# Hippogriff/parsenet-codebase

Measured on AMD Instinct MI355X. Metric: shapes/sec fwd+bwd on 10k-pt clouds, higher is better.
Workload: dtype f32; 1 GPU; cfg5: ParSeNet e2e (seg + mean-shift 10 it. + per-segment spline/primitive fit + Chamfer/residual), 10k pts, batch 4 per GPU, fwd+bwd+allreduce+Adam; batch_per_gpu=4, points=10000, k=80, parallelism=dp1, global_batch=4

## Files before the change

### include/parsenet_hip.h

```cpp
#ifndef PARSENET_HIP_H
#define PARSENET_HIP_H

#include <stddef.h>
#include <stdint.h>

#ifdef __cplusplus
extern "C" {
#endif

#define PN_ABI_VERSION 23

#define PN_OK 0
#define PN_ERR_ARG (-1)
#define PN_ERR_HIP (-2)
#define PN_ERR_WORKSPACE (-3)
#define PN_ERR_UNSUPPORTED (-4)

const char* pn_last_error(void);
int pn_abi_version(void);

void pn_prof_enable(int on);
void pn_prof_reset(void);
int pn_prof_count(void);
int pn_prof_get(int i, char* name, int name_len, double* total_ms, long long* calls);
// ... 74 lines not shown
int pn_gemm_x3_f32(const void* img_a, const float* x, const float* bias, int B, int M, int K, int N, float* out,
                   void* workspace, size_t workspace_bytes, void* stream);
int pn_gemm_x3_cat_f32(const void* img_a, const float* const* xs, const int* cs, int nsrc, const float* bias, int B,
                       int M, int N, float* out, void* workspace, size_t workspace_bytes, void* stream);
size_t pn_gemm_x3_wgrad_workspace(int B, int M, int K, int N);
int pn_gemm_x3_wgrad_f32(const float* gy, const float* x, int B, int M, int K, int N, float* gw, float* gb,
                         void* workspace, size_t workspace_bytes, void* stream);
size_t pn_meanshift_rows_bwd_workspace(int B, int N);
int pn_meanshift_rows_bwd_f32(const float* gy, const float* y, const float* q, const float* rsum, const float* unorm,
                              const float* x, const float* bsq, int B, int N, int D, int R, float* gq, float* gx,
                              void* workspace, size_t workspace_bytes, void* stream);
int pn_meanshift_rows_bwd_kind_f32(const float* gy, const float* y, const float* q, const float* rsum,
                                   const float* unorm, const float* x, const float* bsq, int B, int N, int D, int R,
                                   float* gq, float* gx, void* workspace, size_t workspace_bytes, int kind,
                                   void* stream);
int pn_meanshift_rows_scatter_add_f32(const float* g, const int64_t* rows, int B, int N, int D, int R, float* gx,
                                      void* stream);
size_t pn_meanshift_x3_plan_bytes(int B, int N);
size_t pn_meanshift_x3_plan_core_bytes(int B, int N);
int pn_kmeans_assign_f32(const float* x, const float* cen, int B, int N, int D, int K, int* lab, void* stream);
int pn_kmeans_centres_f32(const float* x, const int* lab, const float* old, int B, int N, int D, int K,
                          float* cen, void* stream);
int pn_cell_order_i32(const int* rank, const int* home, const int* fine, int B, int N, int P, int F,
                      long long* perm, void* stream);
int pn_meanshift_x3_tileinfo_f32(const float* z, int B, int N, int D, float* cen, float* rho, float* cnt,
                                 void* stream);
int pn_meanshift_x3_plan_f32(const float* cenQ, const float* rhoQ, const float* cenX, const float* rhoX,
                             const float* cntX, const float* bsq, int B, int N, float rel_eps, void* plan,
                             void* stream);
int pn_meanshift_x3_iter_fwd_plan_f32(const float* q, const void* img_x, const float* bsq, int B, int N,
// ... 226 lines not shown
```

### parsenet_codebase_amd/csrc/meanshift_rows.hip

```cpp
#include "common.h"
#include <cstdlib>

#define MR_DMAX 128
#define MR_R 64
#define MR_CB 64
#define MR_LDOF(D) ((D) + 4)
#define MR_LG 68
#define MR_LOG2E 1.4426950408889634f
#define MR_LIM2 (75.0f * MR_LOG2E)

__device__ static inline float4 mr_ld4(const float* p) { return *reinterpret_cast<const float4*>(p); }
template <int NV>
__device__ static inline void mr_ldn(const float* p, float* v) {
  if constexpr (NV == 8) {
    const float4 a = mr_ld4(p), b = mr_ld4(p + 4);
    v[0] = a.x; v[1] = a.y; v[2] = a.z; v[3] = a.w;
    v[4] = b.x; v[5] = b.y; v[6] = b.z; v[7] = b.w;
  } else if constexpr (NV == 4) {
    const float4 a = mr_ld4(p);
    v[0] = a.x; v[1] = a.y; v[2] = a.z; v[3] = a.w;
  } else {
    const float2 a = *reinterpret_cast<const float2*>(p);
    v[0] = a.x; v[1] = a.y;
  }
}

template <int MR_D, int MR_LD>
__global__ __launch_bounds__(256) void pn_ms_rows_prep_kernel(const float* __restrict__ gy, const float* __restrict__ y,
                                                              const float* __restrict__ rsum, const float* __restrict__ unorm,
                                                              const float* __restrict__ bsq, int R, float* __restrict__ gu,
                                                              float* __restrict__ scal) {
  const int b = blockIdx.y;
  const int wave = threadIdx.x >> 6, lane = threadIdx.x & 63;
  const int r = blockIdx.x * 4 + wave;
  if (r >= MR_R) return;
  float u0 = 0.f, u1 = 0.f, c = 0.f, al = 0.f, ri = 0.f;
  if (r < R) {
    const size_t base = ((size_t)b * R + r) * MR_D;
    const bool lo = MR_D >= 64 || lane < MR_D;
    float y0 = 0.f, y1 = 0.f, g0 = 0.f, g1 = 0.f;
    if (lo) y0 = y[base + lane];
    if constexpr (MR_D == 128) y1 = y[base + lane + 64];
    if (lo) g0 = gy[base + lane];
    if constexpr (MR_D == 128) g1 = gy[base + lane + 64];
    const float nn = unorm[(size_t)b * R + r], rr = rsum[(size_t)b * R + r];
    const float yg = pn_wave_sum(y0 * g0 + y1 * g1);
    u0 = (g0 - y0 * yg) / nn;
    u1 = (g1 - y1 * yg) / nn;
    c = pn_wave_sum(u0 * (y0 * nn) + u1 * (y1 * nn));
    al = 1.0f / (rr * bsq[b]);
    ri = 1.0f / rr;
  }
  float* g = gu + ((size_t)b * MR_R + r) * MR_D;
  if (lane < MR_D) g[lane] = u0;
  if constexpr (MR_D == 128) g[lane + 64] = u1;
  if (lane == 0) {
    float* sp = scal + ((size_t)b * MR_R + r) * 4;
    sp[0] = c;
    sp[1] = al;
    sp[2] = ri;
    sp[3] = 0.f;
  }
}

template <int MR_D, int MR_LD, int MR_KIND>
__global__ __launch_bounds__(256) void pn_ms_rows_bwd_kernel(
    const float* __restrict__ gu, const float* __restrict__ scal, const float* __restrict__ q,
    const float* __restrict__ x, const float* __restrict__ bsq, int N, int R, int nblk, float* __restrict__ gx,
    float* __restrict__ gq_part) {
  extern __shared__ __attribute__((aligned(16))) float lds[];
  float* Xs = lds;
  float* Qs = Xs + MR_CB * MR_LD;
  float* Us = Qs + MR_R * MR_LD;
  float* GS = Us + MR_R * MR_LD;
  float* KR = GS + MR_R * MR_LG;
  float* GT = KR + MR_R * MR_LG;
  float* sc = GT + MR_CB * MR_LG;
  float* sa = sc + MR_R;
  float* sr = sa + MR_R;
  const int b = blockIdx.y, blk = blockIdx.x, tid = threadIdx.x;
  constexpr int MR_L4 = MR_D == 128 ? 5 : MR_D == 64 ? 4 : 3;

  const int j0 = blk * MR_CB;
  const float bs = bsq[b];
  const float hl = (0.5f / bs) * MR_LOG2E;
  const float ib = 1.0f / bs;
  const float* __restrict__ xb = x + (size_t)b * N * MR_D;

  for (int it = tid; it < MR_CB * (MR_D / 4); it += 256) {
    const int r = it >> MR_L4, c4 = it & (MR_D / 4 - 1);
    float4 v = make_float4(0.f, 0.f, 0.f, 0.f);
    if (j0 + r < N) v = mr_ld4(xb + (size_t)(j0 + r) * MR_D + 4 * c4);
    *reinterpret_cast<float4*>(Xs + r * MR_LD + 4 * c4) = v;
    float4 w = make_float4(0.f, 0.f, 0.f, 0.f);
    if (r < R) w = mr_ld4(q + ((size_t)b * R + r) * MR_D + 4 * c4);
    *reinterpret_cast<float4*>(Qs + r * MR_LD + 4 * c4) = w;
  }
  for (int it = tid; it < MR_R * (MR_D / 4); it += 256) {
    const int r = it >> MR_L4, c4 = it & (MR_D / 4 - 1);
    *reinterpret_cast<float4*>(Us + r * MR_LD + 4 * c4) = mr_ld4(gu + ((size_t)b * MR_R + r) * MR_D + 4 * c4);
  }
  if (tid < MR_R) {
    const float4 sv = mr_ld4(scal + ((size_t)b * MR_R + tid) * 4);
    sc[tid] = sv.x;
    sa[tid] = sv.y;
    sr[tid] = sv.z;
  }
  __syncthreads();

  {
    const int ti = tid >> 4, tj = tid & 15;
    float s[4][4], t[4][4];
#pragma unroll
    for (int a = 0; a < 4; ++a)
#pragma unroll
      for (int e = 0; e < 4; ++e) {
        s[a][e] = 0.f;
        t[a][e] = 0.f;
      }
    for (int k = 0; k < MR_D; k += 4) {
      float4 qv[4], uv[4], xv[4];
#pragma unroll
      for (int a = 0; a < 4; ++a) {
        qv[a] = mr_ld4(Qs + (ti + 16 * a) * MR_LD + k);
        uv[a] = mr_ld4(Us + (ti + 16 * a) * MR_LD + k);
        xv[a] = mr_ld4(Xs + (tj + 16 * a) * MR_LD + k);
      }
#pragma unroll
      for (int a = 0; a < 4; ++a)
#pragma unroll
        for (int e = 0; e < 4; ++e) {
          s[a][e] = __builtin_fmaf(qv[a].x, xv[e].x, s[a][e]);
          s[a][e] = __builtin_fmaf(qv[a].y, xv[e].y, s[a][e]);
          s[a][e] = __builtin_fmaf(qv[a].z, xv[e].z, s[a][e]);
          s[a][e] = __builtin_fmaf(qv[a].w, xv[e].w, s[a][e]);
          t[a][e] = __builtin_fmaf(uv[a].x, xv[e].x, t[a][e]);
          t[a][e] = __builtin_fmaf(uv[a].y, xv[e].y, t[a][e]);
          t[a][e] = __builtin_fmaf(uv[a].z, xv[e].z, t[a][e]);
          t[a][e] = __builtin_fmaf(uv[a].w, xv[e].w, t[a][e]);
        }
    }
#pragma unroll
    for (int a = 0; a < 4; ++a) {
      const int i = ti + 16 * a;
      const float ci = sc[i], ai = sa[i], ri = sr[i];
#pragma unroll
      for (int e = 0; e < 4; ++e) {
        const int j = tj + 16 * e;
        const float dist = __builtin_fmaf(-2.0f, s[a][e], 2.0f);
        float kv, g;
        if constexpr (MR_KIND == PN_MS_KERNEL_EPANECHNIKOV) {
          kv = fmaxf(0.0f, 0.75f * __builtin_fmaf(-dist, ib, 1.0f));
          if (j0 + j >= N) kv = 0.f;
          g = kv > 0.0f ? 1.5f * ((t[a][e] - ci) * ai) : 0.f;
        } else {
          const float a2 = -dist * hl;
          const float a2c = __builtin_amdgcn_fmed3f(a2, -MR_LIM2, MR_LIM2);
          kv = __builtin_amdgcn_exp2f(a2c);
          if (j0 + j >= N) kv = 0.f;
          g = a2c == a2 ? kv * ((t[a][e] - ci) * ai) : 0.f;
        }
        GS[i * MR_LG + j] = g;
        GT[j * MR_LG + i] = g;
        KR[i * MR_LG + j] = kv * ri;
      }
    }
  }
  __syncthreads();

  constexpr int NF4 = MR_D / 4;
  constexpr int RPT = MR_CB * NF4 / 256;
  const int f4 = tid & (NF4 - 1), grp = tid >> MR_L4;
  {
    float4 acc[RPT];
#pragma unroll
    for (int e = 0; e < RPT; ++e) acc[e] = make_float4(0.f, 0.f, 0.f, 0.f);
    for (int i = 0; i < MR_R; ++i) {
      const float4 qv = mr_ld4(Qs + i * MR_LD + 4 * f4);
      const float4 uv = mr_ld4(Us + i * MR_LD + 4 * f4);
      float gv[RPT], kv[RPT];
      mr_ldn<RPT>(GS + i * MR_LG + RPT * grp, gv);
      mr_ldn<RPT>(KR + i * MR_LG + RPT * grp, kv);
#pragma unroll
      for (int e = 0; e < RPT; ++e) {
        acc[e].x = __builtin_fmaf(gv[e], qv.x, acc[e].x);
        acc[e].y = __builtin_fmaf(gv[e], qv.y, acc[e].y);
        acc[e].z = __builtin_fmaf(gv[e], qv.z, acc[e].z);
        acc[e].w = __builtin_fmaf(gv[e], qv.w, acc[e].w);
        acc[e].x = __builtin_fmaf(kv[e], uv.x, acc[e].x);
        acc[e].y = __builtin_fmaf(kv[e], uv.y, acc[e].y);
        acc[e].z = __builtin_fmaf(kv[e], uv.z, acc[e].z);
        acc[e].w = __builtin_fmaf(kv[e], uv.w, acc[e].w);
      }
    }
#pragma unroll
    for (int e = 0; e < RPT; ++e) {
      const int j = j0 + RPT * grp + e;
      if (j < N) {
        float4* o = reinterpret_cast<float4*>(gx + ((size_t)b * N + j) * MR_D + 4 * f4);
        float4 v = *o;
        v.x += acc[e].x;
        v.y += acc[e].y;
        v.z += acc[e].z;
        v.w += acc[e].w;
        *o = v;
      }
    }
  }
  {
    float4 acc[RPT];
#pragma unroll
    for (int e = 0; e < RPT; ++e) acc[e] = make_float4(0.f, 0.f, 0.f, 0.f);
    for (int j = 0; j < MR_CB; ++j) {
      const float4 xv = mr_ld4(Xs + j * MR_LD + 4 * f4);
      float gv[RPT];
      mr_ldn<RPT>(GT + j * MR_LG + RPT * grp, gv);
#pragma unroll
      for (int e = 0; e < RPT; ++e) {
        acc[e].x = __builtin_fmaf(gv[e], xv.x, acc[e].x);
        acc[e].y = __builtin_fmaf(gv[e], xv.y, acc[e].y);
        acc[e].z = __builtin_fmaf(gv[e], xv.z, acc[e].z);
        acc[e].w = __builtin_fmaf(gv[e], xv.w, acc[e].w);
      }
    }
    float* pb = gq_part + ((size_t)b * nblk + blk) * MR_R * MR_D;
#pragma unroll
    for (int e = 0; e < RPT; ++e) *reinterpret_cast<float4*>(pb + (RPT * grp + e) * MR_D + 4 * f4) = acc[e];
  }
}

template <int MR_D, int MR_LD>
__global__ __launch_bounds__(256) void pn_ms_rows_reduce_kernel(const float* __restrict__ gq_part, int R, int nblk,
                                                                float* __restrict__ gq) {
  const int b = blockIdx.y;
  const int e = blockIdx.x * 256 + threadIdx.x;
  if (e >= R * (MR_D / 4)) return;
  const float* p = gq_part + (size_t)b * nblk * MR_R * MR_D + 4 * e;
  float4 s = make_float4(0.f, 0.f, 0.f, 0.f);
  int k = 0;
  for (; k + 8 <= nblk; k += 8) {
    float4 v[8];
#pragma unroll
    for (int u = 0; u < 8; ++u) v[u] = mr_ld4(p + (size_t)(k + u) * MR_R * MR_D);
#pragma unroll
    for (int u = 0; u < 8; ++u) {
      s.x += v[u].x;
      s.y += v[u].y;
      s.z += v[u].z;
      s.w += v[u].w;
    }
  }
  for (; k < nblk; ++k) {
    const float4 v = mr_ld4(p + (size_t)k * MR_R * MR_D);
    s.x += v.x;
    s.y += v.y;
    s.z += v.z;
    s.w += v.w;
  }
  *reinterpret_cast<float4*>(gq + (size_t)b * R * MR_D + 4 * e) = s;
}

template <int MR_D, int MR_LD>
__global__ __launch_bounds__(256) void pn_ms_rows_scatter_kernel(const float* __restrict__ g, const int64_t* __restrict__ rows,
                                                                 int N, int R, float* __restrict__ gx) {
  const int b = blockIdx.x, tid = threadIdx.x;
  const int f4 = tid & 31, sub = tid >> 5;
  for (int r0 = 0; r0 < R; r0 += 8) {
    for (int turn = 0; turn < 8; ++turn) {
      const int r = r0 + turn;
      if (sub == turn && r < R && f4 < MR_D / 4) {
        const int64_t row = rows[(size_t)b * R + r];
        if (row >= 0 && row < N) {
          float4* o = reinterpret_cast<float4*>(gx + ((size_t)b * N + row) * MR_D + 4 * f4);
          const float4 v = mr_ld4(g + ((size_t)b * R + r) * MR_D + 4 * f4);
// ... 6 lines not shown
        }
      }
      __syncthreads();
    }
  }
}

static size_t mr_part_bytes(int B, int N) {
  return pn_align_up((size_t)B * pn_cdiv(N, MR_CB) * MR_R * MR_DMAX * sizeof(float), 256);
}
static size_t mr_gu_bytes(int B) { return pn_align_up((size_t)B * MR_R * MR_DMAX * sizeof(float), 256); }
extern "C" size_t pn_meanshift_rows_bwd_workspace(int B, int N) {
  return mr_part_bytes(B, N) + mr_gu_bytes(B) + pn_align_up((size_t)B * MR_R * 4 * sizeof(float), 256);
}

template <int MR_D, int MR_KIND>
static int mr_rows_bwd(const float* gy, const float* y, const float* q, const float* rsum, const float* unorm,
                       const float* x, const float* bsq, int B, int N, int R, float* gq, float* gx, void* workspace,
                       hipStream_t stream) {
  constexpr int MR_LD = MR_LDOF(MR_D);
  const int nblk = pn_cdiv(N, MR_CB);
  const size_t lds_valu = (size_t)(3 * MR_R * MR_LD + 3 * MR_R * MR_LG + 3 * MR_R) * sizeof(float);
  static unsigned attr_devs = 0;
  if (pn_first_on_device(&attr_devs)) {
    PN_CHECK_HIP(hipFuncSetAttribute(reinterpret_cast<const void*>(pn_ms_rows_bwd_kernel<MR_D, MR_LD, MR_KIND>),
                                     hipFuncAttributeMaxDynamicSharedMemorySize, (int)lds_valu));
  }
  float* part = static_cast<float*>(workspace);
  float* gu = reinterpret_cast<float*>(static_cast<char*>(workspace) + mr_part_bytes(B, N));
  float* scal = reinterpret_cast<float*>(static_cast<char*>(workspace) + mr_part_bytes(B, N) + mr_gu_bytes(B));
  {
    PN_PROF("meanshift_rows_bwd", stream);
    hipLaunchKernelGGL((pn_ms_rows_prep_kernel<MR_D, MR_LD>), dim3(MR_R / 4, B), dim3(256), 0, stream, gy, y, rsum, unorm,
                       bsq, R, gu, scal);
    hipLaunchKernelGGL((pn_ms_rows_bwd_kernel<MR_D, MR_LD, MR_KIND>), dim3(nblk, B), dim3(256), lds_valu, stream, (const float*)gu,
                       (const float*)scal, q, x, bsq, N, R, nblk, gx, part);
  }
  PN_CHECK_LAUNCH();
  hipLaunchKernelGGL((pn_ms_rows_reduce_kernel<MR_D, MR_LD>), dim3(pn_cdiv(R * (MR_D / 4), 256), B), dim3(256), 0, stream,
                     (const float*)part, R, nblk, gq);
  PN_CHECK_LAUNCH();
  return PN_OK;
}

extern "C" int pn_meanshift_rows_bwd_kind_f32(const float* gy, const float* y, const float* q, const float* rsum,
                                              const float* unorm, const float* x, const float* bsq, int B, int N, int D,
                                              int R, float* gq, float* gx, void* workspace, size_t workspace_bytes,
                                              int kind, void* stream_) {
  hipStream_t stream = (hipStream_t)stream_;
  PN_CHECK_ARG(D == 32 || D == 64 || D == 128, "pn_meanshift_rows_bwd_f32: D must be one of {32, 64, 128}, got %d", D);
  PN_CHECK_ARG(R >= 1 && R <= MR_R, "pn_meanshift_rows_bwd_f32: 1 <= R <= %d, got %d", MR_R, R);
  PN_CHECK_ARG(B >= 1 && N >= 1, "pn_meanshift_rows_bwd_f32: empty input");
  PN_CHECK_ARG(kind == PN_MS_KERNEL_GAUSSIAN || kind == PN_MS_KERNEL_EPANECHNIKOV,
               "pn_meanshift_rows_bwd_kind_f32: kernel kind %d unknown (0 Gaussian, 1 Epanechnikov)", kind);
  if (workspace_bytes < pn_meanshift_rows_bwd_workspace(B, N)) {
    pn_set_error("pn_meanshift_rows_bwd_f32: workspace too small");
    return PN_ERR_WORKSPACE;
  }
#define MR_CALL(D_, K_) mr_rows_bwd<D_, K_>(gy, y, q, rsum, unorm, x, bsq, B, N, R, gq, gx, workspace, stream)
  if (kind == PN_MS_KERNEL_EPANECHNIKOV) {
    if (D == 32) return MR_CALL(32, PN_MS_KERNEL_EPANECHNIKOV);
    if (D == 64) return MR_CALL(64, PN_MS_KERNEL_EPANECHNIKOV);
    return MR_CALL(128, PN_MS_KERNEL_EPANECHNIKOV);
  }
  if (D == 32) return MR_CALL(32, PN_MS_KERNEL_GAUSSIAN);
  if (D == 64) return MR_CALL(64, PN_MS_KERNEL_GAUSSIAN);
  return MR_CALL(128, PN_MS_KERNEL_GAUSSIAN);
#undef MR_CALL
}

extern "C" int pn_meanshift_rows_bwd_f32(const float* gy, const float* y, const float* q, const float* rsum,
                                         const float* unorm, const float* x, const float* bsq, int B, int N, int D,
                                         int R, float* gq, float* gx, void* workspace, size_t workspace_bytes,
                                         void* stream_) {
  return pn_meanshift_rows_bwd_kind_f32(gy, y, q, rsum, unorm, x, bsq, B, N, D, R, gq, gx, workspace, workspace_bytes,
                                        PN_MS_KERNEL_GAUSSIAN, stream_);
}

extern "C" int pn_meanshift_rows_scatter_add_f32(const float* g, const int64_t* rows, int B, int N, int D, int R,
                                                 float* gx, void* stream_) {
  hipStream_t stream = (hipStream_t)stream_;
  PN_CHECK_ARG(D == 32 || D == 64 || D == 128, "pn_meanshift_rows_scatter_add_f32: D must be one of {32, 64, 128}, got %d",
               D);
  PN_CHECK_ARG(B >= 1 && R >= 1, "pn_meanshift_rows_scatter_add_f32: empty input");
  if (D == 32)
    hipLaunchKernelGGL((pn_ms_rows_scatter_kernel<32, MR_LDOF(32)>), dim3(B), dim3(256), 0, stream, g, rows, N, R, gx);
  else if (D == 64)
    hipLaunchKernelGGL((pn_ms_rows_scatter_kernel<64, MR_LDOF(64)>), dim3(B), dim3(256), 0, stream, g, rows, N, R, gx);
  else
    hipLaunchKernelGGL((pn_ms_rows_scatter_kernel<128, MR_LDOF(128)>), dim3(B), dim3(256), 0, stream, g, rows, N, R, gx);
  PN_CHECK_LAUNCH();
// ... 3 lines not shown
```

### parsenet_codebase_amd/fitting_batch.py

```python
import os

import numpy as np
import torch
from torch.profiler import record_function

from . import kernels as K
from . import mean_shift as MSM
from ._lib import _PinnedRing, h2d, pinned_like, wait_event
from .dp import FitStatusError
from .losses import normalized_rows

EPS = float(np.finfo(np.float32).eps)
SPLINE_TYPES = (0, 2, 6, 7, 9, 8)
CLOSED_TYPES = (0, 9, 6, 7)
OPEN_TYPES = (2, 8)
PRIM_CODE = {1: K.PRIM_PLANE, 5: K.PRIM_SPHERE, 4: K.PRIM_CYLINDER, 3: K.PRIM_CONE}
PRIM_NAME = {K.PRIM_PLANE: "plane", K.PRIM_SPHERE: "sphere", K.PRIM_CYLINDER: "cylinder", K.PRIM_CONE: "cone"}
CMAX = 64
ROWS_BWD = os.environ.get("PARSENET_MS_ROWS_BWD", "1") != "0"
SPLINE_STREAMS = os.environ.get("PARSENET_SPLINE_STREAMS", "1") != "0"
CALLS_STAGE = {"batched": 0, "per_shape": 0}
CALLS_MEMBERSHIP = {"fused": 0, "tensor": 0}
MEMBERSHIP_WIDTHS = (32, 64, 128)
_SIDE = {}
# ... 446 lines not shown
        for _ in range(B):
            np.random.shuffle(np.arange(N))
        gt_pre = [precompute_ground_truth(labels[b], primitives[b]) for b in range(B)]
        pack = collect(pending)
        if pack[0] > 0:
            MSM.auto_report(B, N, (float(pack[0]) - 1.0) * 1e-6)
        if int(pack[-2 * B:-B].max()) > state["width"]:
            state = cluster(None)
            pack = download(state)
        nms_width_update(ev, B, N, int(pack[-2 * B:-B].max()))
        o = 1
        lab_h = pack[o:o + B * N].reshape(B, N); o += B * N
        cid_h = pack[o:o + B * CMAX].reshape(B, CMAX); o += B * CMAX
        ncl_h, bwflag_h = pack[o:o + B], pack[o + B:o + 2 * B]
        nflag_h = pack[-B:]
        predrawn = all(nflag_h[b] == 0 and bwflag_h[b] == 0 and ncl_h[b] <= 49 for b in range(B))
        if not predrawn:
            np.random.set_state(rng_state)
    else:
        predrawn = False
        gt_pre = [None] * B
        yield
    centers, bws, cluster_ids = [], [], []
    all_fast = state is not None
    for b in range(B):
        fast = state is not None and nflag_h[b] == 0 and bwflag_h[b] == 0 and ncl_h[b] <= CMAX
        if fast and not predrawn:
            np.random.shuffle(np.arange(N))
        if fast and ncl_h[b] <= 49:
            CALLS_STAGE["batched"] += 1
# ... 201 lines not shown
```

### parsenet_codebase_amd/kernels.py

```python
import torch

from . import _lib
from ._lib import check, current_stream, ptr, require_cuda


def _f32c(t, name):
    if t.dtype != torch.float32:
        raise TypeError("%s must be float32, got %s" % (name, t.dtype))
    return t.contiguous()


def chamfer_nn(a, b, side_a=True, side_b=True):
    require_cuda(a, b)
    a = _f32c(a, "a")
    b = _f32c(b, "b")
    if a.dim() != 3 or b.dim() != 3 or a.shape[2] != 3 or b.shape[2] != 3 or a.shape[0] != b.shape[0]:
        raise ValueError("chamfer_nn expects (B,Na,3) and (B,Nb,3), got %s and %s"
                         % (tuple(a.shape), tuple(b.shape)))
    B, Na, _ = a.shape
    Nb = b.shape[1]
    if Na == 0 or Nb == 0 or B == 0:
        raise ValueError("chamfer_nn: empty cloud")
    lib = _lib.load()
    dev = a.device
# ... 715 lines not shown
        raise ValueError("meanshift_rows_bwd: gy, y, q must be (B,R,D)")
    if tuple(rsum.shape) != (B, R) or tuple(unorm.shape) != (B, R) or tuple(gx.shape) != (B, N, D):
        raise ValueError("meanshift_rows_bwd: rsum, unorm (B,R), gx (B,N,D)")
    if gx.dtype != torch.float32 or not gx.is_contiguous():
        raise TypeError("meanshift_rows_bwd: gx must be contiguous fp32")
    lib = _lib.load()
    wsz = lib.pn_meanshift_rows_bwd_workspace(B, N)
    if ws is None or ws.numel() < wsz:
        ws = torch.empty(wsz, dtype=torch.uint8, device=x.device)
    gq = torch.empty_like(q)
    with _lib.on_device(x.device):
        rc = lib.pn_meanshift_rows_bwd_kind_f32(ptr(gy), ptr(y), ptr(q), ptr(rsum), ptr(unorm), ptr(x), ptr(bsq), B, N,
                                                D, R, ptr(gq), ptr(gx), ptr(ws), ws.numel(), int(kind),
                                                current_stream(x.device))
    check(rc, "pn_meanshift_rows_bwd_kind_f32")
    return gq


def meanshift_rows_workspace(B, N, device):
    return torch.empty(_lib.load().pn_meanshift_rows_bwd_workspace(B, N), dtype=torch.uint8, device=device)


def meanshift_rows_scatter_add(gx, rows, g):
    require_cuda(gx, rows, g)
    g = _f32c(g, "g")
    rows = _i64c(rows, "rows")
    B, N, D = gx.shape
    R = rows.shape[1]
    if tuple(g.shape) != (B, R, D) or gx.dtype != torch.float32 or not gx.is_contiguous():
        raise ValueError("meanshift_rows_scatter_add: g (B,R,D), gx contiguous fp32 (B,N,D)")
# ... 500 lines not shown
```

### parsenet_codebase_amd/mean_shift.py

```python
import os
from typing import NamedTuple

import numpy as np
import torch

from . import kernels as K
from ._lib import h2d, require_cuda


ARITH = os.environ.get("PARSENET_MS_ARITH", "bf16x3")
_env_sparse = os.environ.get("PARSENET_MS_SPARSE", "auto")
SPARSE = True if _env_sparse == "1" else False if _env_sparse == "0" else "auto"
AUTO_DENSE_ABOVE = 0.93
AUTO_DENSE_STEPS = 48
AUTO_SAMPLES = 4
_AUTO = {}
CALLS = {"planned": 0, "dense": 0}
AUTO_STAT = None
PLAN_REL_EPS = float(os.environ.get("PARSENET_MS_REL_EPS", "1e-6"))
PLAN_REL_EPS_DENSE_BWD = float(os.environ.get("PARSENET_MS_REL_EPS_BWD", str(min(PLAN_REL_EPS, 1e-9))))
SPARSE_MIN_N = 2048
SPARSE_MAX_N = 32768
LAST_PLAN_STATS = None
WANT_NEAREST = False
# ... 330 lines not shown

class _CentreRows(torch.autograd.Function):

    @staticmethod
    def forward(ctx, X, state, ids):
        B, N, D = state.x.shape
        T = state.iterations
        ids = ids.long()
        rows = torch.gather(state.inv, 1, ids) if state.inv is not None else ids
        R = rows.shape[1]
        Qc = torch.gather(state.iterates, 2, rows.view(1, B, R, 1).expand(T + 1, B, R, D))
        rc = torch.gather(state.rsums, 2, rows.view(1, B, R).expand(T, B, R))
        nc = torch.gather(state.norms, 2, rows.view(1, B, R).expand(T, B, R))
        ctx.T, ctx.kind = T, state.kind
        ctx.has_inv = state.inv is not None
        ctx.save_for_backward(Qc, rc, nc, rows, state.x, state.bsq, *([state.inv] if state.inv is not None else []))
        return Qc[T].clone()

    @staticmethod
    def backward(ctx, g):
        Qc, rc, nc, rows, x, bsq = ctx.saved_tensors[:6]
        B, N, D = x.shape
        gX = torch.zeros_like(x)
        g = g.contiguous()
        ws = K.meanshift_rows_workspace(B, N, x.device)
        for t in reversed(range(ctx.T)):
            g = K.meanshift_rows_bwd(g, Qc[t + 1], Qc[t], rc[t], nc[t], x, bsq, gX, ws, kind=ctx.kind)
        K.meanshift_rows_scatter_add(gX, rows, g)
        if ctx.has_inv:
            inv = ctx.saved_tensors[6]
            gX = torch.gather(gX, 1, inv.unsqueeze(2).expand(-1, -1, D))
        return gX, None, None


def centre_rows(X, state, ids):
    if state.kind != K.KERNEL_GAUSSIAN:
        _require_fused_epanechnikov("centre_rows", X)
    if ids.shape[1] > 64:
        raise ValueError("centre_rows: at most 64 rows per batch item, got %d" % ids.shape[1])
    return _CentreRows.apply(X, state, ids)


def _first_argmax(vals, dim):
    m = vals.max(dim, keepdim=True)[0]
    n = vals.shape[dim]
    shape = [1] * vals.dim()
    shape[dim] = n
    ar = torch.arange(n, device=vals.device).view(shape)
    return torch.where(vals == m, ar, torch.full_like(ar, n)).min(dim)[0]


class MeanShift:
    def __init__(self):
        pass

# ... 136 lines not shown
```

Measured before the change: 179.5 shapes/s.

## Chain mean-shift row backward over iterations and skip unused centre rows

Replaces the per-iteration Python loop of mean-shift row backward calls with one chained native entry point that walks all T iterations, fusing the partial-gradient reduce with the next iteration's prep kernel. The row kernel is templated on a padded row count, so when fewer centre rows are in use (set from the fitting stage via the autograd node), it loads and computes only those rows and uses a smaller LDS footprint for higher occupancy. This cuts launch and host overhead and wasted FLOPs on padded rows. It adds more template instantiations and a side channel that sets rows_in_use on the grad_fn node, which has to be correct or the gradients will be wrong.

```diff
diff --git a/include/parsenet_hip.h b/include/parsenet_hip.h
--- a/include/parsenet_hip.h
+++ b/include/parsenet_hip.h
@@ -112,6 +112,10 @@
                                    const float* unorm, const float* x, const float* bsq, int B, int N, int D, int R,
                                    float* gq, float* gx, void* workspace, size_t workspace_bytes, int kind,
                                    void* stream);
+int pn_meanshift_rows_bwd_chain_kind_f32(const float* gy, const float* qc, const float* rsum, const float* unorm,
+                                         const float* x, const float* bsq, int B, int N, int D, int R, int rows_used,
+                                         int T, float* gq, float* gx, void* workspace, size_t workspace_bytes, int kind,
+                                         void* stream);
 int pn_meanshift_rows_scatter_add_f32(const float* g, const int64_t* rows, int B, int N, int D, int R, float* gx,
                                       void* stream);
 size_t pn_meanshift_x3_plan_bytes(int B, int N);
diff --git a/parsenet_codebase_amd/csrc/meanshift_rows.hip b/parsenet_codebase_amd/csrc/meanshift_rows.hip
--- a/parsenet_codebase_amd/csrc/meanshift_rows.hip
+++ b/parsenet_codebase_amd/csrc/meanshift_rows.hip
@@ -6,8 +6,11 @@
 #define MR_CB 64
 #define MR_LDOF(D) ((D) + 4)
 #define MR_LG 68
+#define MR_LGTOF(RP) ((RP) + 4)
 #define MR_LOG2E 1.4426950408889634f
 #define MR_LIM2 (75.0f * MR_LOG2E)
+#define MR_LDS_FLOATS(D, RP) (MR_CB * MR_LDOF(D) + 2 * (RP) * MR_LDOF(D) + 2 * (RP) * MR_LG + MR_CB * MR_LGTOF(RP) + 3 * (RP))
+#define MR_WGS(D, RP) ((RP) == MR_R ? 1 : (160 * 1024 / (MR_LDS_FLOATS(D, RP) * 4) < 4 ? 160 * 1024 / (MR_LDS_FLOATS(D, RP) * 4) : 4))
 
 __device__ static inline float4 mr_ld4(const float* p) { return *reinterpret_cast<const float4*>(p); }
 template <int NV>
@@ -19,37 +22,40 @@
   } else if constexpr (NV == 4) {
     const float4 a = mr_ld4(p);
     v[0] = a.x; v[1] = a.y; v[2] = a.z; v[3] = a.w;
+  } else if constexpr (NV == 2 || NV == 6) {
+#pragma unroll
+    for (int e = 0; e < NV; e += 2) {
+      const float2 a = *reinterpret_cast<const float2*>(p + e);
+      v[e] = a.x; v[e + 1] = a.y;
+    }
   } else {
-    const float2 a = *reinterpret_cast<const float2*>(p);
-    v[0] = a.x; v[1] = a.y;
-  }
-}
-
-template <int MR_D, int MR_LD>
-__global__ __launch_bounds__(256) void pn_ms_rows_prep_kernel(const float* __restrict__ gy, const float* __restrict__ y,
-                                                              const float* __restrict__ rsum, const float* __restrict__ unorm,
-                                                              const float* __restrict__ bsq, int R, float* __restrict__ gu,
-                                                              float* __restrict__ scal) {
-  const int b = blockIdx.y;
-  const int wave = threadIdx.x >> 6, lane = threadIdx.x & 63;
-  const int r = blockIdx.x * 4 + wave;
-  if (r >= MR_R) return;
+#pragma unroll
+    for (int e = 0; e < NV; ++e) v[e] = p[e];
+  }
+}
+
+__device__ static inline void mr_prep_row(float g0, float g1, float y0, float y1, float nn, float rr, float bs, float& u0,
+                                          float& u1, float& c, float& al, float& ri) {
+  const float yg = pn_wave_sum(y0 * g0 + y1 * g1);
+  u0 = (g0 - y0 * yg) / nn;
+  u1 = (g1 - y1 * yg) / nn;
+  c = pn_wave_sum(u0 * (y0 * nn) + u1 * (y1 * nn));
+  al = 1.0f / (rr * bs);
+  ri = 1.0f / rr;
+}
+template <int MR_D>
+__device__ static inline void mr_prep_store(float g0, float g1, const float* __restrict__ y, const float* __restrict__ rsum,
+                                            const float* __restrict__ unorm, const float* __restrict__ bsq, int b, int r,
+                                            int R, int RU, int lane, float* __restrict__ gu, float* __restrict__ scal) {
   float u0 = 0.f, u1 = 0.f, c = 0.f, al = 0.f, ri = 0.f;
-  if (r < R) {
+  if (r < RU) {
     const size_t base = ((size_t)b * R + r) * MR_D;
     const bool lo = MR_D >= 64 || lane < MR_D;
-    float y0 = 0.f, y1 = 0.f, g0 = 0.f, g1 = 0.f;
+    float y0 = 0.f, y1 = 0.f;
     if (lo) y0 = y[base + lane];
     if constexpr (MR_D == 128) y1 = y[base + lane + 64];
-    if (lo) g0 = gy[base + lane];
-    if constexpr (MR_D == 128) g1 = gy[base + lane + 64];
     const float nn = unorm[(size_t)b * R + r], rr = rsum[(size_t)b * R + r];
-    const float yg = pn_wave_sum(y0 * g0 + y1 * g1);
-    u0 = (g0 - y0 * yg) / nn;
-    u1 = (g1 - y1 * yg) / nn;
-    c = pn_wave_sum(u0 * (y0 * nn) + u1 * (y1 * nn));
-    al = 1.0f / (rr * bsq[b]);
-    ri = 1.0f / rr;
+    mr_prep_row(g0, g1, y0, y1, nn, rr, bsq[b], u0, u1, c, al, ri);
   }
   float* g = gu + ((size_t)b * MR_R + r) * MR_D;
   if (lane < MR_D) g[lane] = u0;
@@ -63,21 +69,92 @@
   }
 }
 
-template <int MR_D, int MR_LD, int MR_KIND>
-__global__ __launch_bounds__(256) void pn_ms_rows_bwd_kernel(
+template <int MR_D, int MR_LD>
+__global__ __launch_bounds__(256) void pn_ms_rows_prep_kernel(const float* __restrict__ gy, const float* __restrict__ y,
+                                                              const float* __restrict__ rsum, const float* __restrict__ unorm,
+                                                              const float* __restrict__ bsq, int R, int RU,
+                                                              float* __restrict__ gu, float* __restrict__ scal) {
+  const int b = blockIdx.y;
+  const int wave = threadIdx.x >> 6, lane = threadIdx.x & 63;
+  const int r = blockIdx.x * 4 + wave;
+  if (r >= MR_R) return;
+  float g0 = 0.f, g1 = 0.f;
+  if (r < RU) {
+    const size_t base = ((size_t)b * R + r) * MR_D;
+    if (MR_D >= 64 || lane < MR_D) g0 = gy[base + lane];
+    if constexpr (MR_D == 128) g1 = gy[base + lane + 64];
+  }
+  mr_prep_store<MR_D>(g0, g1, y, rsum, unorm, bsq, b, r, R, RU, lane, gu, scal);
+}
+
+#define MR_DOTS_BODY \
+      float4 qv[NA], uv[NA], xv[4]; \
+_Pragma("unroll") \
+      for (int a = 0; a < NA; ++a) { \
+        qv[a] = mr_ld4(Qs + (ti + 16 * a) * MR_LD + k); \
+        uv[a] = mr_ld4(Us + (ti + 16 * a) * MR_LD + k); \
+      } \
+_Pragma("unroll") \
+      for (int e = 0; e < 4; ++e) xv[e] = mr_ld4(Xs + (tj + 16 * e) * MR_LD + k); \
+_Pragma("unroll") \
+      for (int a = 0; a < NA; ++a) \
+_Pragma("unroll") \
+        for (int e = 0; e < 4; ++e) { \
+          s[a][e] = __builtin_fmaf(qv[a].x, xv[e].x, s[a][e]); \
+          s[a][e] = __builtin_fmaf(qv[a].y, xv[e].y, s[a][e]); \
+          s[a][e] = __builtin_fmaf(qv[a].z, xv[e].z, s[a][e]); \
+          s[a][e] = __builtin_fmaf(qv[a].w, xv[e].w, s[a][e]); \
+          t[a][e] = __builtin_fmaf(uv[a].x, xv[e].x, t[a][e]); \
+          t[a][e] = __builtin_fmaf(uv[a].y, xv[e].y, t[a][e]); \
+          t[a][e] = __builtin_fmaf(uv[a].z, xv[e].z, t[a][e]); \
+          t[a][e] = __builtin_fmaf(uv[a].w, xv[e].w, t[a][e]); \
+        }
+#define MR_ROW_BODY \
+      const float4 qv = mr_ld4(Qs + i * MR_LD + 4 * f4); \
+      const float4 uv = mr_ld4(Us + i * MR_LD + 4 * f4); \
+      float gv[RPT], kv[RPT]; \
+      mr_ldn<RPT>(GS + i * MR_LG + RPT * grp, gv); \
+      mr_ldn<RPT>(KR + i * MR_LG + RPT * grp, kv); \
+_Pragma("unroll") \
+      for (int e = 0; e < RPT; ++e) { \
+        acc[e].x = __builtin_fmaf(gv[e], qv.x, acc[e].x); \
+        acc[e].y = __builtin_fmaf(gv[e], qv.y, acc[e].y); \
+        acc[e].z = __builtin_fmaf(gv[e], qv.z, acc[e].z); \
+        acc[e].w = __builtin_fmaf(gv[e], qv.w, acc[e].w); \
+        acc[e].x = __builtin_fmaf(kv[e], uv.x, acc[e].x); \
+        acc[e].y = __builtin_fmaf(kv[e], uv.y, acc[e].y); \
+        acc[e].z = __builtin_fmaf(kv[e], uv.z, acc[e].z); \
+        acc[e].w = __builtin_fmaf(kv[e], uv.w, acc[e].w); \
+      }
+#define MR_COL_BODY \
+        const float4 xv = mr_ld4(Xs + j * MR_LD + 4 * f4); \
+        float gv[RQ]; \
+        mr_ldn<RQ>(GT + j * MR_LGT + RQ * grp, gv); \
+_Pragma("unroll") \
+        for (int e = 0; e < RQ; ++e) { \
+          acc[e].x = __builtin_fmaf(gv[e], xv.x, acc[e].x); \
+          acc[e].y = __builtin_fmaf(gv[e], xv.y, acc[e].y); \
+          acc[e].z = __builtin_fmaf(gv[e], xv.z, acc[e].z); \
+          acc[e].w = __builtin_fmaf(gv[e], xv.w, acc[e].w); \
+        }
+
+template <int MR_D, int MR_LD, int MR_KIND, int MR_RP>
+__global__ __launch_bounds__(256, MR_WGS(MR_D, MR_RP)) void pn_ms_rows_bwd_kernel(
     const float* __restrict__ gu, const float* __restrict__ scal, const float* __restrict__ q,
-    const float* __restrict__ x, const float* __restrict__ bsq, int N, int R, int nblk, float* __restrict__ gx,
+    const float* __restrict__ x, const float* __restrict__ bsq, int N, int R, int RU, int nblk, float* __restrict__ gx,
     float* __restrict__ gq_part) {
+  static_assert(MR_RP % 16 == 0 && MR_RP >= 16 && MR_RP <= MR_R, "MR_RP: 16, 32, 48 or 64");
+  constexpr int MR_LGT = MR_LGTOF(MR_RP);
   extern __shared__ __attribute__((aligned(16))) float lds[];
   float* Xs = lds;
   float* Qs = Xs + MR_CB * MR_LD;
-  float* Us = Qs + MR_R * MR_LD;
-  float* GS = Us + MR_R * MR_LD;
-  float* KR = GS + MR_R * MR_LG;
-  float* GT = KR + MR_R * MR_LG;
-  float* sc = GT + MR_CB * MR_LG;
-  float* sa = sc + MR_R;
-  float* sr = sa + MR_R;
+  float* Us = Qs + MR_RP * MR_LD;
+  float* GS = Us + MR_RP * MR_LD;
+  float* KR = GS + MR_RP * MR_LG;
+  float* GT = KR + MR_RP * MR_LG;
+  float* sc = GT + MR_CB * MR_LGT;
+  float* sa = sc + MR_RP;
+  float* sr = sa + MR_RP;
   const int b = blockIdx.y, blk = blockIdx.x, tid = threadIdx.x;
   constexpr int MR_L4 = MR_D == 128 ? 5 : MR_D == 64 ? 4 : 3;
 
@@ -92,15 +169,17 @@
     float4 v = make_float4(0.f, 0.f, 0.f, 0.f);
     if (j0 + r < N) v = mr_ld4(xb + (size_t)(j0 + r) * MR_D + 4 * c4);
     *reinterpret_cast<float4*>(Xs + r * MR_LD + 4 * c4) = v;
-    float4 w = make_float4(0.f, 0.f, 0.f, 0.f);
-    if (r < R) w = mr_ld4(q + ((size_t)b * R + r) * MR_D + 4 * c4);
-    *reinterpret_cast<float4*>(Qs + r * MR_LD + 4 * c4) = w;
-  }
-  for (int it = tid; it < MR_R * (MR_D / 4); it += 256) {
+    if (MR_RP == MR_CB || r < MR_RP) {
+      float4 w = make_float4(0.f, 0.f, 0.f, 0.f);
+      if (r < RU) w = mr_ld4(q + ((size_t)b * R + r) * MR_D + 4 * c4);
+      *reinterpret_cast<float4*>(Qs + r * MR_LD + 4 * c4) = w;
+    }
+  }
+  for (int it = tid; it < MR_RP * (MR_D / 4); it += 256) {
     const int r = it >> MR_L4, c4 = it & (MR_D / 4 - 1);
     *reinterpret_cast<float4*>(Us + r * MR_LD + 4 * c4) = mr_ld4(gu + ((size_t)b * MR_R + r) * MR_D + 4 * c4);
   }
-  if (tid < MR_R) {
+  if (tid < MR_RP) {
     const float4 sv = mr_ld4(scal + ((size_t)b * MR_R + tid) * 4);
     sc[tid] = sv.x;
     sa[tid] = sv.y;
@@ -109,39 +188,28 @@
   __syncthreads();
 
   {
+    constexpr int NA = MR_RP / 16;
     const int ti = tid >> 4, tj = tid & 15;
-    float s[4][4], t[4][4];
-#pragma unroll
-    for (int a = 0; a < 4; ++a)
+    float s[NA][4], t[NA][4];
+#pragma unroll
+    for (int a = 0; a < NA; ++a)
 #pragma unroll
       for (int e = 0; e < 4; ++e) {
         s[a][e] = 0.f;
         t[a][e] = 0.f;
       }
-    for (int k = 0; k < MR_D; k += 4) {
-      float4 qv[4], uv[4], xv[4];
-#pragma unroll
-      for (int a = 0; a < 4; ++a) {
-        qv[a] = mr_ld4(Qs + (ti + 16 * a) * MR_LD + k);
-        uv[a] = mr_ld4(Us + (ti + 16 * a) * MR_LD + k);
-        xv[a] = mr_ld4(Xs + (tj + 16 * a) * MR_LD + k);
-      }
-#pragma unroll
-      for (int a = 0; a < 4; ++a)
-#pragma unroll
-        for (int e = 0; e < 4; ++e) {
-          s[a][e] = __builtin_fmaf(qv[a].x, xv[e].x, s[a][e]);
-          s[a][e] = __builtin_fmaf(qv[a].y, xv[e].y, s[a][e]);
-          s[a][e] = __builtin_fmaf(qv[a].z, xv[e].z, s[a][e]);
-          s[a][e] = __builtin_fmaf(qv[a].w, xv[e].w, s[a][e]);
-          t[a][e] = __builtin_fmaf(uv[a].x, xv[e].x, t[a][e]);
-          t[a][e] = __builtin_fmaf(uv[a].y, xv[e].y, t[a][e]);
-          t[a][e] = __builtin_fmaf(uv[a].z, xv[e].z, t[a][e]);
-          t[a][e] = __builtin_fmaf(uv[a].w, xv[e].w, t[a][e]);
-        }
-    }
-#pragma unroll
-    for (int a = 0; a < 4; ++a) {
+    if constexpr (MR_RP == MR_R) {
+      for (int k = 0; k < MR_D; k += 4) {
+        MR_DOTS_BODY
+      }
+    } else {
+#pragma unroll 2
+      for (int k = 0; k < MR_D; k += 4) {
+        MR_DOTS_BODY
+      }
+    }
+#pragma unroll
+    for (int a = 0; a < NA; ++a) {
       const int i = ti + 16 * a;
       const float ci = sc[i], ai = sa[i], ri = sr[i];
 #pragma unroll
@@ -161,7 +229,7 @@
           g = a2c == a2 ? kv * ((t[a][e] - ci) * ai) : 0.f;
         }
         GS[i * MR_LG + j] = g;
-        GT[j * MR_LG + i] = g;
+        GT[j * MR_LGT + i] = g;
         KR[i * MR_LG + j] = kv * ri;
       }
     }
@@ -175,22 +243,14 @@
     float4 acc[RPT];
 #pragma unroll
     for (int e = 0; e < RPT; ++e) acc[e] = make_float4(0.f, 0.f, 0.f, 0.f);
-    for (int i = 0; i < MR_R; ++i) {
-      const float4 qv = mr_ld4(Qs + i * MR_LD + 4 * f4);
-      const float4 uv = mr_ld4(Us + i * MR_LD + 4 * f4);
-      float gv[RPT], kv[RPT];
-      mr_ldn<RPT>(GS + i * MR_LG + RPT * grp, gv);
-      mr_ldn<RPT>(KR + i * MR_LG + RPT * grp, kv);
-#pragma unroll
-      for (int e = 0; e < RPT; ++e) {
-        acc[e].x = __builtin_fmaf(gv[e], qv.x, acc[e].x);
-        acc[e].y = __builtin_fmaf(gv[e], qv.y, acc[e].y);
-        acc[e].z = __builtin_fmaf(gv[e], qv.z, acc[e].z);
-        acc[e].w = __builtin_fmaf(gv[e], qv.w, acc[e].w);
-        acc[e].x = __builtin_fmaf(kv[e], uv.x, acc[e].x);
-        acc[e].y = __builtin_fmaf(kv[e], uv.y, acc[e].y);
-        acc[e].z = __builtin_fmaf(kv[e], uv.z, acc[e].z);
-        acc[e].w = __builtin_fmaf(kv[e], uv.w, acc[e].w);
+    if constexpr (MR_RP == MR_R) {
+      for (int i = 0; i < MR_RP; ++i) {
+        MR_ROW_BODY
+      }
+    } else {
+#pragma unroll 4
+      for (int i = 0; i < MR_RP; ++i) {
+        MR_ROW_BODY
       }
     }
 #pragma unroll
@@ -208,56 +268,72 @@
     }
   }
   {
-    float4 acc[RPT];
-#pragma unroll
-    for (int e = 0; e < RPT; ++e) acc[e] = make_float4(0.f, 0.f, 0.f, 0.f);
-    for (int j = 0; j < MR_CB; ++j) {
-      const float4 xv = mr_ld4(Xs + j * MR_LD + 4 * f4);
-      float gv[RPT];
-      mr_ldn<RPT>(GT + j * MR_LG + RPT * grp, gv);
-#pragma unroll
-      for (int e = 0; e < RPT; ++e) {
-        acc[e].x = __builtin_fmaf(gv[e], xv.x, acc[e].x);
-        acc[e].y = __builtin_fmaf(gv[e], xv.y, acc[e].y);
-        acc[e].z = __builtin_fmaf(gv[e], xv.z, acc[e].z);
-        acc[e].w = __builtin_fmaf(gv[e], xv.w, acc[e].w);
-      }
-    }
-    float* pb = gq_part + ((size_t)b * nblk + blk) * MR_R * MR_D;
-#pragma unroll
-    for (int e = 0; e < RPT; ++e) *reinterpret_cast<float4*>(pb + (RPT * grp + e) * MR_D + 4 * f4) = acc[e];
-  }
-}
-
+    constexpr int NG = 256 / NF4;
+    constexpr int RQ = (MR_RP + NG - 1) / NG;
+    if (RQ * NG == MR_RP || RQ * grp < MR_RP) {
+      float4 acc[RQ];
+#pragma unroll
+      for (int e = 0; e < RQ; ++e) acc[e] = make_float4(0.f, 0.f, 0.f, 0.f);
+      if constexpr (MR_RP == MR_R) {
+        for (int j = 0; j < MR_CB; ++j) {
+          MR_COL_BODY
+        }
+      } else {
+#pragma unroll 4
+        for (int j = 0; j < MR_CB; ++j) {
+          MR_COL_BODY
+        }
+      }
+      float* pb = gq_part + ((size_t)b * nblk + blk) * MR_R * MR_D;
+#pragma unroll
+      for (int e = 0; e < RQ; ++e) *reinterpret_cast<float4*>(pb + (RQ * grp + e) * MR_D + 4 * f4) = acc[e];
+    }
+  }
+}
+
+#define MR_RED 16
 template <int MR_D, int MR_LD>
-__global__ __launch_bounds__(256) void pn_ms_rows_reduce_kernel(const float* __restrict__ gq_part, int R, int nblk,
-                                                                float* __restrict__ gq) {
+__global__ __launch_bounds__(256) void pn_ms_rows_reduce_prep_kernel(
+    const float* __restrict__ gq_part, int R, int RU, int nblk, float* __restrict__ gq, const float* __restrict__ y,
+    const float* __restrict__ rsum, const float* __restrict__ unorm, const float* __restrict__ bsq,
+    float* __restrict__ gu, float* __restrict__ scal) {
   const int b = blockIdx.y;
-  const int e = blockIdx.x * 256 + threadIdx.x;
-  if (e >= R * (MR_D / 4)) return;
-  const float* p = gq_part + (size_t)b * nblk * MR_R * MR_D + 4 * e;
-  float4 s = make_float4(0.f, 0.f, 0.f, 0.f);
-  int k = 0;
-  for (; k + 8 <= nblk; k += 8) {
-    float4 v[8];
-#pragma unroll
-    for (int u = 0; u < 8; ++u) v[u] = mr_ld4(p + (size_t)(k + u) * MR_R * MR_D);
-#pragma unroll
-    for (int u = 0; u < 8; ++u) {
-      s.x += v[u].x;
-      s.y += v[u].y;
-      s.z += v[u].z;
-      s.w += v[u].w;
-    }
-  }
-  for (; k < nblk; ++k) {
-    const float4 v = mr_ld4(p + (size_t)k * MR_R * MR_D);
-    s.x += v.x;
-    s.y += v.y;
-    s.z += v.z;
-    s.w += v.w;
-  }
-  *reinterpret_cast<float4*>(gq + (size_t)b * R * MR_D + 4 * e) = s;
+  const int wave = threadIdx.x >> 6, lane = threadIdx.x & 63;
+  const int r = blockIdx.x * 4 + wave;
+  if (r >= MR_R) return;
+  const bool lo = MR_D >= 64 || lane < MR_D;
+  float g0 = 0.f, g1 = 0.f;
+  if (r < RU) {
+    constexpr size_t STEP = (size_t)MR_R * MR_D;
+    const float* p = gq_part + ((size_t)b * nblk * MR_R + r) * MR_D + (lo ? lane : 0);
+    float s0 = 0.f, s1 = 0.f;
+    int k = 0;
+    for (; k + MR_RED <= nblk; k += MR_RED) {
+      float v0[MR_RED], v1[MR_RED];
+#pragma unroll
+      for (int u = 0; u < MR_RED; ++u) {
+        v0[u] = p[(size_t)(k + u) * STEP];
+        if constexpr (MR_D == 128) v1[u] = p[(size_t)(k + u) * STEP + 64];
+      }
+#pragma unroll
+      for (int u = 0; u < MR_RED; ++u) {
+        s0 += v0[u];
+        if constexpr (MR_D == 128) s1 += v1[u];
+      }
+    }
+    for (; k < nblk; ++k) {
+      s0 += p[(size_t)k * STEP];
+      if constexpr (MR_D == 128) s1 += p[(size_t)k * STEP + 64];
+    }
+    if (lo) g0 = s0;
+    g1 = s1;
+  }
+  if (gq != nullptr && r < R) {
+    float* o = gq + ((size_t)b * R + r) * MR_D;
+    if (lane < MR_D) o[lane] = g0;
+    if constexpr (MR_D == 128) o[lane + 64] = g1;
+  }
+  if (y != nullptr) mr_prep_store<MR_D>(g0, g1, y, rsum, unorm, bsq, b, r, R, RU, lane, gu, scal);
 }
 
 template <int MR_D, int MR_LD>
@@ -294,59 +370,88 @@
   return mr_part_bytes(B, N) + mr_gu_bytes(B) + pn_align_up((size_t)B * MR_R * 4 * sizeof(float), 256);
 }
 
-template <int MR_D, int MR_KIND>
-static int mr_rows_bwd(const float* gy, const float* y, const float* q, const float* rsum, const float* unorm,
-                       const float* x, const float* bsq, int B, int N, int R, float* gq, float* gx, void* workspace,
-                       hipStream_t stream) {
+struct MrChain {
+  const float *gy, *y_top, *qc, *rsum, *unorm, *x, *bsq;
+  int B, N, R, RU, T;
+  float *gq, *gx;
+  void* workspace;
+  hipStream_t stream;
+};
+
+template <int MR_D, int MR_KIND, int MR_RP>
+static int mr_launch_bwd(const MrChain& a, const float* gu, const float* scal, const float* q, float* part) {
   constexpr int MR_LD = MR_LDOF(MR_D);
-  const int nblk = pn_cdiv(N, MR_CB);
-  const size_t lds_valu = (size_t)(3 * MR_R * MR_LD + 3 * MR_R * MR_LG + 3 * MR_R) * sizeof(float);
+  constexpr size_t lds_valu = (size_t)MR_LDS_FLOATS(MR_D, MR_RP) * sizeof(float);
   static unsigned attr_devs = 0;
   if (pn_first_on_device(&attr_devs)) {
-    PN_CHECK_HIP(hipFuncSetAttribute(reinterpret_cast<const void*>(pn_ms_rows_bwd_kernel<MR_D, MR_LD, MR_KIND>),
+    PN_CHECK_HIP(hipFuncSetAttribute(reinterpret_cast<const void*>(pn_ms_rows_bwd_kernel<MR_D, MR_LD, MR_KIND, MR_RP>),
                                      hipFuncAttributeMaxDynamicSharedMemorySize, (int)lds_valu));
   }
-  float* part = static_cast<float*>(workspace);
-  float* gu = reinterpret_cast<float*>(static_cast<char*>(workspace) + mr_part_bytes(B, N));
-  float* scal = reinterpret_cast<float*>(static_cast<char*>(workspace) + mr_part_bytes(B, N) + mr_gu_bytes(B));
-  {
-    PN_PROF("meanshift_rows_bwd", stream);
-    hipLaunchKernelGGL((pn_ms_rows_prep_kernel<MR_D, MR_LD>), dim3(MR_R / 4, B), dim3(256), 0, stream, gy, y, rsum, unorm,
-                       bsq, R, gu, scal);
-    hipLaunchKernelGGL((pn_ms_rows_bwd_kernel<MR_D, MR_LD, MR_KIND>), dim3(nblk, B), dim3(256), lds_valu, stream, (const float*)gu,
-                       (const float*)scal, q, x, bsq, N, R, nblk, gx, part);
-  }
-  PN_CHECK_LAUNCH();
-  hipLaunchKernelGGL((pn_ms_rows_reduce_kernel<MR_D, MR_LD>), dim3(pn_cdiv(R * (MR_D / 4), 256), B), dim3(256), 0, stream,
-                     (const float*)part, R, nblk, gq);
-  PN_CHECK_LAUNCH();
+  const int nblk = pn_cdiv(a.N, MR_CB);
+  hipLaunchKernelGGL((pn_ms_rows_bwd_kernel<MR_D, MR_LD, MR_KIND, MR_RP>), dim3(nblk, a.B), dim3(256), lds_valu, a.stream, gu,
+                     scal, q, a.x, a.bsq, a.N, a.R, a.RU, nblk, a.gx, part);
   return PN_OK;
+}
+
+template <int MR_D, int MR_KIND>
+static int mr_rows_chain(const MrChain& a) {
+  constexpr int MR_LD = MR_LDOF(MR_D);
+  const int nblk = pn_cdiv(a.N, MR_CB);
+  const size_t rows = (size_t)a.B * a.R;
+  float* part = static_cast<float*>(a.workspace);
+  float* gu = reinterpret_cast<float*>(static_cast<char*>(a.workspace) + mr_part_bytes(a.B, a.N));
+  float* scal = reinterpret_cast<float*>(static_cast<char*>(a.workspace) + mr_part_bytes(a.B, a.N) + mr_gu_bytes(a.B));
+  for (int t = a.T - 1; t >= 0; --t) {
+    const float* q = a.qc + (size_t)t * rows * MR_D;
+    {
+      PN_PROF("meanshift_rows_bwd", a.stream);
+      if (t == a.T - 1)
+        hipLaunchKernelGGL((pn_ms_rows_prep_kernel<MR_D, MR_LD>), dim3(MR_R / 4, a.B), dim3(256), 0, a.stream, a.gy, a.y_top,
+                           a.rsum + (size_t)t * rows, a.unorm + (size_t)t * rows, a.bsq, a.R, a.RU, gu, scal);
+      int rc;
+      if (a.RU <= 16) rc = mr_launch_bwd<MR_D, MR_KIND, 16>(a, gu, scal, q, part);
+      else if (a.RU <= 32) rc = mr_launch_bwd<MR_D, MR_KIND, 32>(a, gu, scal, q, part);
+      else if (a.RU <= 48) rc = mr_launch_bwd<MR_D, MR_KIND, 48>(a, gu, scal, q, part);
+      else rc = mr_launch_bwd<MR_D, MR_KIND, 64>(a, gu, scal, q, part);
+      if (rc != PN_OK) return rc;
+    }
+    PN_CHECK_LAUNCH();
+    hipLaunchKernelGGL((pn_ms_rows_reduce_prep_kernel<MR_D, MR_LD>), dim3(MR_R / 4, a.B), dim3(256), 0, a.stream,
+                       (const float*)part, a.R, a.RU, nblk, t == 0 ? a.gq : (float*)nullptr, t > 0 ? q : (const float*)nullptr,
+                       t > 0 ? a.rsum + (size_t)(t - 1) * rows : (const float*)nullptr,
+                       t > 0 ? a.unorm + (size_t)(t - 1) * rows : (const float*)nullptr, a.bsq, gu, scal);
+    PN_CHECK_LAUNCH();
+  }
+  return PN_OK;
+}
+
+static int mr_dispatch(const char* who, const MrChain& a, int D, size_t workspace_bytes, int kind) {
+  PN_CHECK_ARG(D == 32 || D == 64 || D == 128, "pn_meanshift_rows_bwd_f32: D must be one of {32, 64, 128}, got %d", D);
+  PN_CHECK_ARG(a.R >= 1 && a.R <= MR_R, "pn_meanshift_rows_bwd_f32: 1 <= R <= %d, got %d", MR_R, a.R);
+  PN_CHECK_ARG(a.RU >= 1 && a.RU <= a.R, "%s: 1 <= rows in use <= R = %d, got %d", who, a.R, a.RU);
+  PN_CHECK_ARG(a.B >= 1 && a.N >= 1 && a.T >= 1, "pn_meanshift_rows_bwd_f32: empty input");
+  PN_CHECK_ARG(kind == PN_MS_KERNEL_GAUSSIAN || kind == PN_MS_KERNEL_EPANECHNIKOV,
+               "pn_meanshift_rows_bwd_kind_f32: kernel kind %d unknown (0 Gaussian, 1 Epanechnikov)", kind);
+  if (workspace_bytes < pn_meanshift_rows_bwd_workspace(a.B, a.N)) {
+    pn_set_error("pn_meanshift_rows_bwd_f32: workspace too small");
+    return PN_ERR_WORKSPACE;
+  }
+  if (kind == PN_MS_KERNEL_EPANECHNIKOV) {
+    if (D == 32) return mr_rows_chain<32, PN_MS_KERNEL_EPANECHNIKOV>(a);
+    if (D == 64) return mr_rows_chain<64, PN_MS_KERNEL_EPANECHNIKOV>(a);
+    return mr_rows_chain<128, PN_MS_KERNEL_EPANECHNIKOV>(a);
+  }
+  if (D == 32) return mr_rows_chain<32, PN_MS_KERNEL_GAUSSIAN>(a);
+  if (D == 64) return mr_rows_chain<64, PN_MS_KERNEL_GAUSSIAN>(a);
+  return mr_rows_chain<128, PN_MS_KERNEL_GAUSSIAN>(a);
 }
 
 extern "C" int pn_meanshift_rows_bwd_kind_f32(const float* gy, const float* y, const float* q, const float* rsum,
                                               const float* unorm, const float* x, const float* bsq, int B, int N, int D,
                                               int R, float* gq, float* gx, void* workspace, size_t workspace_bytes,
                                               int kind, void* stream_) {
-  hipStream_t stream = (hipStream_t)stream_;
-  PN_CHECK_ARG(D == 32 || D == 64 || D == 128, "pn_meanshift_rows_bwd_f32: D must be one of {32, 64, 128}, got %d", D);
-  PN_CHECK_ARG(R >= 1 && R <= MR_R, "pn_meanshift_rows_bwd_f32: 1 <= R <= %d, got %d", MR_R, R);
-  PN_CHECK_ARG(B >= 1 && N >= 1, "pn_meanshift_rows_bwd_f32: empty input");
-  PN_CHECK_ARG(kind == PN_MS_KERNEL_GAUSSIAN || kind == PN_MS_KERNEL_EPANECHNIKOV,
-               "pn_meanshift_rows_bwd_kind_f32: kernel kind %d unknown (0 Gaussian, 1 Epanechnikov)", kind);
-  if (workspace_bytes < pn_meanshift_rows_bwd_workspace(B, N)) {
-    pn_set_error("pn_meanshift_rows_bwd_f32: workspace too small");
-    return PN_ERR_WORKSPACE;
-  }
-#define MR_CALL(D_, K_) mr_rows_bwd<D_, K_>(gy, y, q, rsum, unorm, x, bsq, B, N, R, gq, gx, workspace, stream)
-  if (kind == PN_MS_KERNEL_EPANECHNIKOV) {
-    if (D == 32) return MR_CALL(32, PN_MS_KERNEL_EPANECHNIKOV);
-    if (D == 64) return MR_CALL(64, PN_MS_KERNEL_EPANECHNIKOV);
-    return MR_CALL(128, PN_MS_KERNEL_EPANECHNIKOV);
-  }
-  if (D == 32) return MR_CALL(32, PN_MS_KERNEL_GAUSSIAN);
-  if (D == 64) return MR_CALL(64, PN_MS_KERNEL_GAUSSIAN);
-  return MR_CALL(128, PN_MS_KERNEL_GAUSSIAN);
-#undef MR_CALL
+  const MrChain a = {gy, y, q, rsum, unorm, x, bsq, B, N, R, R, 1, gq, gx, workspace, (hipStream_t)stream_};
+  return mr_dispatch("pn_meanshift_rows_bwd_kind_f32", a, D, workspace_bytes, kind);
 }
 
 extern "C" int pn_meanshift_rows_bwd_f32(const float* gy, const float* y, const float* q, const float* rsum,
@@ -355,6 +460,16 @@
                                          void* stream_) {
   return pn_meanshift_rows_bwd_kind_f32(gy, y, q, rsum, unorm, x, bsq, B, N, D, R, gq, gx, workspace, workspace_bytes,
                                         PN_MS_KERNEL_GAUSSIAN, stream_);
+}
+
+extern "C" int pn_meanshift_rows_bwd_chain_kind_f32(const float* gy, const float* qc, const float* rsum, const float* unorm,
+                                                    const float* x, const float* bsq, int B, int N, int D, int R,
+                                                    int rows_used, int T, float* gq, float* gx, void* workspace,
+                                                    size_t workspace_bytes, int kind, void* stream_) {
+  PN_CHECK_ARG(T >= 1 && B >= 1 && R >= 1 && D >= 1, "pn_meanshift_rows_bwd_chain_kind_f32: T, B, R >= 1");
+  const MrChain a = {gy, qc + (size_t)T * B * R * D, qc, rsum, unorm, x, bsq, B, N, R, rows_used, T, gq, gx, workspace,
+                     (hipStream_t)stream_};
+  return mr_dispatch("pn_meanshift_rows_bwd_chain_kind_f32", a, D, workspace_bytes, kind);
 }
 
 extern "C" int pn_meanshift_rows_scatter_add_f32(const float* g, const int64_t* rows, int B, int N, int D, int R,
diff --git a/parsenet_codebase_amd/fitting_batch.py b/parsenet_codebase_amd/fitting_batch.py
--- a/parsenet_codebase_amd/fitting_batch.py
+++ b/parsenet_codebase_amd/fitting_batch.py
@@ -484,6 +484,8 @@
         cid_h = pack[o:o + B * CMAX].reshape(B, CMAX); o += B * CMAX
         ncl_h, bwflag_h = pack[o:o + B], pack[o + B:o + 2 * B]
         nflag_h = pack[-B:]
+        if ms_state is not None:
+            MSM.centre_rows_in_use(state["cen"], int(np.clip(ncl_h, 1, CMAX).max()))
         predrawn = all(nflag_h[b] == 0 and bwflag_h[b] == 0 and ncl_h[b] <= 49 for b in range(B))
         if not predrawn:
             np.random.set_state(rng_state)
diff --git a/parsenet_codebase_amd/kernels.py b/parsenet_codebase_amd/kernels.py
--- a/parsenet_codebase_amd/kernels.py
+++ b/parsenet_codebase_amd/kernels.py
@@ -753,6 +753,33 @@
                                                 D, R, ptr(gq), ptr(gx), ptr(ws), ws.numel(), int(kind),
                                                 current_stream(x.device))
     check(rc, "pn_meanshift_rows_bwd_kind_f32")
+    return gq
+
+
+def meanshift_rows_bwd_chain(gy, qc, rsum, unorm, x, bsq, gx, ws=None, kind=KERNEL_GAUSSIAN, rows_used=None):
+    require_cuda(gy, qc, rsum, unorm, x, bsq, gx)
+    gy, qc, x = _f32c(gy, "gy"), _f32c(qc, "qc"), _f32c(x, "x")
+    rsum, unorm, bsq = _f32c(rsum, "rsum"), _f32c(unorm, "unorm"), _f32c(bsq, "bsq")
+    B, N, D = x.shape
+    if gy.dim() != 3 or qc.dim() != 4 or qc.shape[0] < 2:
+        raise ValueError("meanshift_rows_bwd_chain: gy (B,R,D), qc (T+1,B,R,D) with T >= 1")
+    T, R = qc.shape[0] - 1, gy.shape[1]
+    if tuple(gy.shape) != (B, R, D) or tuple(qc.shape) != (T + 1, B, R, D):
+        raise ValueError("meanshift_rows_bwd_chain: gy (B,R,D), qc (T+1,B,R,D)")
+    if tuple(rsum.shape) != (T, B, R) or tuple(unorm.shape) != (T, B, R) or tuple(gx.shape) != (B, N, D):
+        raise ValueError("meanshift_rows_bwd_chain: rsum, unorm (T,B,R), gx (B,N,D)")
+    if gx.dtype != torch.float32 or not gx.is_contiguous():
+        raise TypeError("meanshift_rows_bwd_chain: gx must be contiguous fp32")
+    lib = _lib.load()
+    wsz = lib.pn_meanshift_rows_bwd_workspace(B, N)
+    if ws is None or ws.numel() < wsz:
+        ws = torch.empty(wsz, dtype=torch.uint8, device=x.device)
+    gq = torch.empty_like(gy)
+    with _lib.on_device(x.device):
+        rc = lib.pn_meanshift_rows_bwd_chain_kind_f32(ptr(gy), ptr(qc), ptr(rsum), ptr(unorm), ptr(x), ptr(bsq), B, N, D, R,
+                                                      R if rows_used is None else int(rows_used), T, ptr(gq), ptr(gx),
+                                                      ptr(ws), ws.numel(), int(kind), current_stream(x.device))
+    check(rc, "pn_meanshift_rows_bwd_chain_kind_f32")
     return gq
 
 
diff --git a/parsenet_codebase_amd/mean_shift.py b/parsenet_codebase_amd/mean_shift.py
--- a/parsenet_codebase_amd/mean_shift.py
+++ b/parsenet_codebase_amd/mean_shift.py
@@ -368,6 +368,7 @@
         nc = torch.gather(state.norms, 2, rows.view(1, B, R).expand(T, B, R))
         ctx.T, ctx.kind = T, state.kind
         ctx.has_inv = state.inv is not None
+        ctx.rows_in_use = None
         ctx.save_for_backward(Qc, rc, nc, rows, state.x, state.bsq, *([state.inv] if state.inv is not None else []))
         return Qc[T].clone()
 
@@ -378,8 +379,8 @@
         gX = torch.zeros_like(x)
         g = g.contiguous()
         ws = K.meanshift_rows_workspace(B, N, x.device)
-        for t in reversed(range(ctx.T)):
-            g = K.meanshift_rows_bwd(g, Qc[t + 1], Qc[t], rc[t], nc[t], x, bsq, gX, ws, kind=ctx.kind)
+        if ctx.T > 0:
+            g = K.meanshift_rows_bwd_chain(g, Qc, rc, nc, x, bsq, gX, ws, kind=ctx.kind, rows_used=ctx.rows_in_use)
         K.meanshift_rows_scatter_add(gX, rows, g)
         if ctx.has_inv:
             inv = ctx.saved_tensors[6]
@@ -393,6 +394,12 @@
     if ids.shape[1] > 64:
         raise ValueError("centre_rows: at most 64 rows per batch item, got %d" % ids.shape[1])
     return _CentreRows.apply(X, state, ids)
+
+
+def centre_rows_in_use(centres, n):
+    node = centres.grad_fn
+    if node is not None and hasattr(node, "rows_in_use"):
+        node.rows_in_use = max(1, min(int(n), centres.shape[1]))
 
 
 def _first_argmax(vals, dim):
```

Result: faster. 182.2 shapes/s, median of 6 (+1.5%).
